# tarepan/VectorQuantizedCPC

Hardware: AMD Instinct MI355X
Metric: audio samples/sec (WaveRNN-style decode, convert.py path: encode + generate) (higher is better)
Workload: dtype f32

## Files before the change

### include/vqcpc.h

```cpp
#ifndef VQCPC_H
#define VQCPC_H

#include <stdint.h>

#ifdef __cplusplus
extern "C" {
#endif

#define VQCPC_ABI_VERSION 1

typedef enum {
    VQCPC_OK = 0,
    VQCPC_ERR_INVALID = -1,
    VQCPC_ERR_HIP = -2,
    VQCPC_ERR_NO_DEVICE = -3,
    VQCPC_ERR_ALLOC = -4
} vqcpc_status;

int vqcpc_abi_version(void);
const char *vqcpc_last_error(void);

int vqcpc_device_count(void);


// ... 71 lines not shown
typedef struct vqcpc_vocoder vqcpc_vocoder;

int vqcpc_vocoder_create(const vqcpc_vocoder_weights *w, vqcpc_vocoder **out);
void vqcpc_vocoder_destroy(vqcpc_vocoder *voc);

int vqcpc_vocoder_generate(vqcpc_vocoder *voc, const int64_t *idx, const int64_t *speaker,
                           int B, int Tc, const int *n_codes, uint64_t seed, uint32_t utt_base,
                           const uint32_t *utt_ids, float *wav, int64_t *mulaw, int max_steps,
                           void *stream);

typedef struct vqcpc_vocoder_stream vqcpc_vocoder_stream;
int vqcpc_vocoder_stream_open(vqcpc_vocoder *voc, const int64_t *idx, const int64_t *speaker, int B, int Tc,
                              const int *n_codes, uint64_t seed, uint32_t utt_base, const uint32_t *utt_ids,
                              vqcpc_vocoder_stream **out, void *stream);
int vqcpc_vocoder_stream_next(vqcpc_vocoder_stream *st, int n_samples, float *wav, int64_t *mulaw, void *stream);
int vqcpc_vocoder_stream_redo(vqcpc_vocoder_stream *st, float *wav, int64_t *mulaw, void *stream);
int vqcpc_vocoder_stream_position(const vqcpc_vocoder_stream *st, int64_t *done, int64_t *total);
void vqcpc_vocoder_stream_close(vqcpc_vocoder_stream *st);

int vqcpc_vocoder_logits(vqcpc_vocoder *voc, const int64_t *x, const int64_t *idx,
                         const int64_t *speaker, int B, int Tc, int Ts, float *logits,
                         void *stream);

int vqcpc_vocoder_nll(vqcpc_vocoder *voc, const int64_t *audio, const int64_t *idx, const int64_t *speaker,
                      int B, int Tc, int L, const int *n_codes, const int *n_audio,
                      double *nll_sum, int64_t *n_scored, int64_t *n_correct, float *nll, void *stream);

int vqcpc_vocoder_glue(vqcpc_vocoder *voc, const int64_t *idx, const int64_t *speaker, int B, int Tc, float *series,
                       void *stream);

int vqcpc_vocoder_condition(vqcpc_vocoder *voc, const int64_t *idx, const int64_t *speaker,
                            int B, int Tc, float *cond, void *stream);

int vqcpc_vocoder_set_option(vqcpc_vocoder *voc, const char *name, int value);

int vqcpc_vocoder_check(vqcpc_vocoder *voc);

int vqcpc_vocoder_last_path(vqcpc_vocoder *voc);

int vqcpc_vocoder_plan(int xcd, int xcm, int xcm_min, int xcm_max, int xcd_slots, int xcm_slots, int slots,
                       const int *n_samples, int B, int *path, int *slots_used, int64_t *longest);

int vqcpc_vocoder_last_slots(vqcpc_vocoder *voc);

int vqcpc_vocoder_workspace_bytes(vqcpc_vocoder *voc, uint64_t *bytes);

int vqcpc_vocoder_last_timing(vqcpc_vocoder *voc, float *loop_ms, int *n_steps);


typedef struct vqcpc_melfront vqcpc_melfront;
int vqcpc_melfront_create(int sr, int n_fft, int n_mels, int hop, int win, float fmin, float preemph,
                          float top_db, vqcpc_melfront **out);
void vqcpc_melfront_destroy(vqcpc_melfront *f);
int vqcpc_melfront_frames(const vqcpc_melfront *f, int n_samples);
int vqcpc_melfront_run(vqcpc_melfront *f, const float *wav, const int *lens, int B, int Lmax, float *mel,
                       void *stream);


typedef struct vqcpc_resampler vqcpc_resampler;
int vqcpc_resampler_create(int sr_in, int sr_out, vqcpc_resampler **out);
void vqcpc_resampler_destroy(vqcpc_resampler *r);
int vqcpc_resampler_out_len(const vqcpc_resampler *r, int n_in);
int vqcpc_resampler_run(vqcpc_resampler *r, const float *wav_in, const int *lens_in, int B, int Lin_max,
                        float *wav_out, int Lout_max, void *stream);


// ... 16 lines not shown
```

### vectorquantizedcpc_amd/_lib.py

```python
import ctypes as C
import os

_HERE = os.path.dirname(os.path.abspath(__file__))
LIB_PATH = os.path.join(_HERE, "libvqcpc_hip.so")

SYMBOLS = [
    "vqcpc_abi_version", "vqcpc_last_error", "vqcpc_device_count",
    "vqcpc_encoder_create", "vqcpc_encoder_destroy", "vqcpc_encoder_encode",
    "vqcpc_encoder_forward_stats", "vqcpc_encoder_context", "vqcpc_encoder_stage", "vqcpc_encoder_vq_encode", "vqcpc_encoder_set_option", "vqcpc_encoder_last_schedule",
    "vqcpc_cpc_create", "vqcpc_cpc_destroy", "vqcpc_cpc_score",
    "vqcpc_encoder_check", "vqcpc_vocoder_check", "vqcpc_vocoder_last_path", "vqcpc_vocoder_last_slots", "vqcpc_vocoder_workspace_bytes", "vqcpc_vocoder_plan",
    "vqcpc_vocoder_create", "vqcpc_vocoder_destroy", "vqcpc_vocoder_generate",
    "vqcpc_vocoder_logits", "vqcpc_vocoder_nll", "vqcpc_vocoder_condition", "vqcpc_vocoder_glue", "vqcpc_vocoder_set_option",
    "vqcpc_vocoder_last_timing", "vqcpc_vocoder_kernel_times",
    "vqcpc_vocoder_stream_open", "vqcpc_vocoder_stream_next", "vqcpc_vocoder_stream_redo", "vqcpc_vocoder_stream_position",
    "vqcpc_vocoder_stream_close",
    "vqcpc_melfront_create", "vqcpc_melfront_destroy", "vqcpc_melfront_frames", "vqcpc_melfront_run",
    "vqcpc_loudness_create", "vqcpc_loudness_destroy", "vqcpc_loudness_blocks", "vqcpc_loudness_integrated",
    "vqcpc_loudness_normalize",
    "vqcpc_resampler_create", "vqcpc_resampler_destroy", "vqcpc_resampler_out_len", "vqcpc_resampler_run",
]


class EncoderWeights(C.Structure):
    _fields_ = [("conv_weight", C.c_void_p), ("ln_weight", C.c_void_p * 5), ("ln_bias", C.c_void_p * 5),
                ("fc_weight", C.c_void_p * 4), ("out_weight", C.c_void_p), ("out_bias", C.c_void_p),
                ("codebook", C.c_void_p), ("rnn_w_ih", C.c_void_p), ("rnn_w_hh", C.c_void_p),
                ("rnn_b_ih", C.c_void_p), ("rnn_b_hh", C.c_void_p),
                ("in_channels", C.c_int), ("channels", C.c_int), ("n_embeddings", C.c_int),
                ("z_dim", C.c_int), ("c_dim", C.c_int)]


class CPCWeights(C.Structure):
    _fields_ = [("weight", C.c_void_p * 16), ("bias", C.c_void_p * 16),
                ("n_steps", C.c_int), ("n_speakers", C.c_int), ("n_utterances", C.c_int), ("n_negatives", C.c_int),
                ("z_dim", C.c_int), ("c_dim", C.c_int)]


class VocoderWeights(C.Structure):
    _fields_ = [("code_embedding", C.c_void_p), ("speaker_embedding", C.c_void_p),
                ("prenet_w_ih", (C.c_void_p * 2) * 2), ("prenet_w_hh", (C.c_void_p * 2) * 2),
                ("prenet_b_ih", (C.c_void_p * 2) * 2), ("prenet_b_hh", (C.c_void_p * 2) * 2),
                ("ar_embedding", C.c_void_p), ("ar_w_ih", C.c_void_p), ("ar_w_hh", C.c_void_p),
                ("ar_b_ih", C.c_void_p), ("ar_b_hh", C.c_void_p),
                ("fc1_weight", C.c_void_p), ("fc1_bias", C.c_void_p), ("fc2_weight", C.c_void_p), ("fc2_bias", C.c_void_p),
                ("n_codes", C.c_int), ("dz", C.c_int), ("n_speakers", C.c_int), ("ds", C.c_int), ("Hp", C.c_int),
# ... 15 lines not shown
    lib = C.CDLL(LIB_PATH)
    vp, i32, i64p = C.c_void_p, C.c_int, C.c_void_p
    lib.vqcpc_abi_version.restype = i32
    lib.vqcpc_last_error.restype = C.c_char_p
    lib.vqcpc_device_count.restype = i32
    lib.vqcpc_encoder_create.argtypes = [C.POINTER(EncoderWeights), C.POINTER(vp)]
    lib.vqcpc_encoder_destroy.argtypes = [vp]
    lib.vqcpc_encoder_destroy.restype = None
    lib.vqcpc_encoder_encode.argtypes = [vp, vp, i32, i32, i32, vp, vp, i64p, vp, vp]
    lib.vqcpc_encoder_forward_stats.argtypes = [vp, vp, vp, i64p, i32, vp, vp, vp, vp]
    lib.vqcpc_encoder_context.argtypes = [vp, vp, i32, i32, vp, vp]
    lib.vqcpc_encoder_stage.argtypes = [vp, vp, i32, i32, i32, i32, vp, vp]
    lib.vqcpc_encoder_vq_encode.argtypes = [vp, vp, i32, vp, i64p, vp]
    lib.vqcpc_encoder_set_option.argtypes = [vp, C.c_char_p, i32]
    lib.vqcpc_encoder_check.argtypes = [vp]
    lib.vqcpc_encoder_last_schedule.argtypes = [vp]
    lib.vqcpc_cpc_create.argtypes = [C.POINTER(CPCWeights), C.POINTER(vp)]
    lib.vqcpc_cpc_destroy.argtypes = [vp]
    lib.vqcpc_cpc_destroy.restype = None
    lib.vqcpc_cpc_score.argtypes = [vp, vp, vp, i32, i64p, i64p, C.c_uint64, C.c_uint32, vp, vp, vp, vp, vp, vp]
    lib.vqcpc_vocoder_check.argtypes = [vp]
    lib.vqcpc_vocoder_last_path.argtypes = [vp]
    lib.vqcpc_vocoder_last_slots.argtypes = [vp]
    lib.vqcpc_vocoder_workspace_bytes.argtypes = [vp, C.POINTER(C.c_uint64)]
    lib.vqcpc_vocoder_plan.argtypes = [i32] * 7 + [C.POINTER(C.c_int), i32, C.POINTER(C.c_int), C.POINTER(C.c_int), C.POINTER(C.c_int64)]
    lib.vqcpc_vocoder_create.argtypes = [C.POINTER(VocoderWeights), C.POINTER(vp)]
    lib.vqcpc_vocoder_destroy.argtypes = [vp]
    lib.vqcpc_vocoder_destroy.restype = None
    lib.vqcpc_vocoder_generate.argtypes = [vp, i64p, i64p, i32, i32, C.POINTER(C.c_int), C.c_uint64, C.c_uint32,
                                           C.POINTER(C.c_uint32), vp, i64p, i32, vp]
    lib.vqcpc_vocoder_logits.argtypes = [vp, i64p, i64p, i64p, i32, i32, i32, vp, vp]
    lib.vqcpc_vocoder_nll.argtypes = [vp, i64p, i64p, i64p, i32, i32, i32, C.POINTER(C.c_int), C.POINTER(C.c_int), vp, i64p, i64p, vp, vp]
    lib.vqcpc_vocoder_condition.argtypes = [vp, i64p, i64p, i32, i32, vp, vp]
    lib.vqcpc_vocoder_glue.argtypes = [vp, i64p, i64p, i32, i32, vp, vp]
    lib.vqcpc_vocoder_set_option.argtypes = [vp, C.c_char_p, i32]
    lib.vqcpc_vocoder_last_timing.argtypes = [vp, C.POINTER(C.c_float), C.POINTER(C.c_int)]
    lib.vqcpc_vocoder_kernel_times.argtypes = [vp, i32, C.POINTER(C.c_float), vp]
    lib.vqcpc_vocoder_stream_open.argtypes = [vp, i64p, i64p, i32, i32, C.POINTER(C.c_int), C.c_uint64, C.c_uint32,
                                              C.POINTER(C.c_uint32), C.POINTER(vp), vp]
    lib.vqcpc_vocoder_stream_next.argtypes = [vp, i32, vp, i64p, vp]
    lib.vqcpc_vocoder_stream_redo.argtypes = [vp, vp, i64p, vp]
    lib.vqcpc_vocoder_stream_position.argtypes = [vp, C.POINTER(C.c_int64), C.POINTER(C.c_int64)]
    lib.vqcpc_vocoder_stream_close.argtypes = [vp]
    lib.vqcpc_vocoder_stream_close.restype = None
    lib.vqcpc_melfront_create.argtypes = [i32, i32, i32, i32, i32, C.c_float, C.c_float, C.c_float, C.POINTER(vp)]
    lib.vqcpc_melfront_destroy.argtypes = [vp]
    lib.vqcpc_melfront_destroy.restype = None
    lib.vqcpc_melfront_frames.argtypes = [vp, i32]
    lib.vqcpc_melfront_run.argtypes = [vp, vp, C.POINTER(C.c_int), i32, i32, vp, vp]
    lib.vqcpc_loudness_create.argtypes = [i32, C.POINTER(vp)]
    lib.vqcpc_loudness_destroy.argtypes = [vp]
    lib.vqcpc_loudness_destroy.restype = None
    lib.vqcpc_loudness_blocks.argtypes = [vp, i32]
    lib.vqcpc_loudness_integrated.argtypes = [vp, vp, C.POINTER(C.c_int), i32, i32, vp, vp, vp]
    lib.vqcpc_loudness_normalize.argtypes = [vp, vp, C.POINTER(C.c_int), i32, i32, vp, vp, vp]
    lib.vqcpc_resampler_create.argtypes = [i32, i32, C.POINTER(vp)]
    lib.vqcpc_resampler_destroy.argtypes = [vp]
    lib.vqcpc_resampler_destroy.restype = None
    lib.vqcpc_resampler_out_len.argtypes = [vp, i32]
    lib.vqcpc_resampler_run.argtypes = [vp, vp, C.POINTER(C.c_int), i32, i32, vp, i32, vp]
    lib.vqcpc_probe_gates.argtypes = [vp, i32, vp, vp]
    _lib = lib
    return lib


def check(rc: int):
# ... 58 lines not shown
```

### vectorquantizedcpc_amd/csrc/common.h

```cpp
#pragma once
#include <hip/hip_runtime.h>
#include <stdint.h>
#include <stddef.h>
#include "../../include/vqcpc.h"

void vq_set_error(const char *fmt, ...) __attribute__((format(printf, 1, 2)));
int vq_require_gfx950();

#define HIP_TRY(expr)                                                                      \
    do {                                                                                   \
        hipError_t e_ = (expr);                                                            \
        if (e_ != hipSuccess) {                                                            \
            vq_set_error("%s failed: %s (%s:%d)", #expr, hipGetErrorString(e_), __FILE__,  \
                         __LINE__);                                                        \
            return VQCPC_ERR_HIP;                                                          \
        }                                                                                  \
    } while (0)

#define VQ_REQUIRE(cond, ...)                   \
    do {                                        \
        if (!(cond)) {                          \
            vq_set_error(__VA_ARGS__);          \
            return VQCPC_ERR_INVALID;           \
        }                                       \
// ... 8 lines not shown
    void *p = nullptr;
    size_t cap = 0;
    int reserve(size_t bytes) {
        if (bytes <= cap) return VQCPC_OK;
        if (p) (void)hipFree(p);
        p = nullptr; cap = 0;
        hipError_t e = hipMalloc(&p, bytes);
        if (e != hipSuccess) {
            vq_set_error("hipMalloc(%zu) failed: %s", bytes, hipGetErrorString(e));
            return VQCPC_ERR_ALLOC;
        }
        cap = bytes;
        return VQCPC_OK;
    }
    void release() { if (p) (void)hipFree(p); p = nullptr; cap = 0; }
    template <class T> T **fresh() { release(); return (T **)&p; }
    template <class T> T *as() const { return (T *)p; }
};
template <class T> struct DevPtr : DevBuf {
    DevPtr() = default;
    DevPtr(const DevPtr &) = delete;
    DevPtr &operator=(const DevPtr &) = delete;
    ~DevPtr() { release(); }
    operator T *() const { return (T *)p; }
};

int vq_gemm_chain(const float *A, int lda, const float *W, const float *bias, float *Y, int ldy,
                  int M, int N, int K, int KC, hipStream_t s);

int vq_gemm_chain_ex(const float *A, int lda, const float *W, const float *bias, float *Y, int ldy,
                     int M, int N, int K, int KC, int relu, int ydiv, int ystride, int yoff, int ylim, hipStream_t s);

int vq_build_wfrag(const float *W, int ldw, int n_rg, int K, int ksplit, int rowmode, int H, float **out);
int vq_bigru_scan(const float *Wf, const float *b_hh, const float *Gi, float *hbuf, float *out, const int *len, const int *row0,
                  int H, int B, int T, hipStream_t s);
struct LstmPlan;
int vq_lstm_plan_create(const float *w_ih, const float *w_hh, const float *b_ih, const float *b_hh,
                        int D, int H, LstmPlan **out);
void vq_lstm_plan_destroy(LstmPlan *p);
int vq_lstm_run(LstmPlan *p, const float *x, int B, int T, float *out, hipStream_t s);
int vq_lstm_set_persistent(LstmPlan *p, int value);
int vq_lstm_set_debug(LstmPlan *p, int drop_step, int timeout_ms);
int vq_lstm_check(LstmPlan *p);
```

### vectorquantizedcpc_amd/csrc/scan.hip

```cpp
#include "common.h"
#include "ar_shared.h"
#include <math.h>

__global__ void build_wfrag_kernel(const float *__restrict__ W, int ldw, float *__restrict__ Wf, int n_rg,
                                   int K, int ksplit, int rowmode, int H) {
    const int SW = K / 16 / ksplit;
    const size_t total = (size_t)n_rg * ksplit * SW * 64;
    const size_t id = (size_t)blockIdx.x * blockDim.x + threadIdx.x;
    if (id >= total) return;
    const int lane = (int)(id & 63);
    size_t r = id >> 6;
    const int s = (int)(r % SW); r /= SW;
    const int w = (int)(r % ksplit);
    const int rg = (int)(r / ksplit);
    const int i = lane & 15, kq = lane >> 4, S = w * SW + s;
    int row;
    if (rowmode == 0) row = 16 * rg + i;
    else if (rowmode == 8) row = i < 8 ? 8 * rg + i : -1;
    else if (rowmode == 16) row = (rg % 3) * H + 16 * (rg / 3) + i;
    else row = (i >> 2) < rowmode ? (i >> 2) * H + 4 * rg + (i & 3) : -1;
    float4 v = make_float4(0.f, 0.f, 0.f, 0.f);
    if (row >= 0) v = *(const float4 *)(W + (size_t)row * ldw + 16 * S + 4 * kq);
    ((float4 *)Wf)[id] = v;
}
// ... 61 lines not shown
    __syncthreads();
    if (act) {
        float hn;
        if (G == 3) {
            const float r = sigmoidf_(g0 + (gate[u][b] + bh0));
            const float z = sigmoidf_(g1 + (gate[4 + u][b] + bh1));
            const float n = tanhf(g2 + r * (gate[8 + u][b] + bh2));
            hn = (1.0f - z) * n + z * hold;
        } else {
            const float ig = sigmoidf_(g0 + gate[u][b]), fg = sigmoidf_(g1 + gate[4 + u][b]);
            const float gg = tanhf(g2 + gate[8 + u][b]), og = sigmoidf_(g3 + gate[12 + u][b]);
            const float cn = fg * cold + ig * gg;
            p.cbuf[(size_t)dir * hsz + hi] = cn;
            hn = og * tanhf(cn);
        }
        hout[hi] = hn;
        p.out[((p.row0 ? (size_t)p.row0[bg] : (size_t)bg * p.T) + tpos) * (p.ndir * H) + (size_t)dir * H + unit] = hn;
    }
}

template <int G>
static int launch_seq(const SeqP &p, int step, hipStream_t s) {
    const int SW = p.H / 64;
    dim3 grid(p.H / 4, p.ndir, p.nbt), blk(256);
    switch (SW) {
#define CASE(n) case n: hipLaunchKernelGGL((seq_step_kernel<G, n>), grid, blk, 0, s, p, step); break;
        CASE(1) CASE(2) CASE(4) CASE(8)
#undef CASE
        default: vq_set_error("recurrent step: hidden size %d unsupported (64, 128, 256 and 512 are built)", p.H); return VQCPC_ERR_INVALID;
    }
    return VQCPC_OK;
}

int vq_bigru_scan(const float *Wf, const float *b_hh, const float *Gi, float *hbuf, float *out, const int *len, const int *row0,
                  int H, int B, int T, hipStream_t s) {
    const int nbt = (B + 15) / 16;
    HIP_TRY(hipMemsetAsync(hbuf, 0, (size_t)2 * 2 * nbt * H * 16 * sizeof(float), s));
    SeqP q{};
    q.Wf = Wf; q.b_hh = b_hh; q.Gi = Gi; q.hbuf = hbuf;
    q.out = out; q.len = len; q.row0 = row0; q.H = H; q.nbt = nbt; q.B = B; q.T = T; q.ndir = 2;
    for (int t = 0; t < T; ++t) TRY(launch_seq<3>(q, t, s));
    return VQCPC_OK;
}

__global__ void add_vec_kernel(const float *a, const float *b, float *o, int n) {
    const int i = blockIdx.x * blockDim.x + threadIdx.x;
    if (i < n) o[i] = a[i] + b[i];
}

struct LstmPlan {
    int D, H;
    float *w_ih = nullptr, *bias = nullptr, *Wf = nullptr;
    float *w_hh = nullptr;
    DevBuf gi, hbuf, cbuf, px;
    unsigned *abort_host = nullptr;
    int persistent = -1;
    bool pending = false;
    int dbg_drop_step = -1;
    int timeout_ms = 1000;
};
static int lstm_persist_launch(LstmPlan *p, int T, float *out, hipStream_t s);
void vq_lstm_plan_destroy(LstmPlan *p) {
    if (!p) return;
    if (p->w_ih) (void)hipFree(p->w_ih);
    if (p->bias) (void)hipFree(p->bias);
    if (p->Wf) (void)hipFree(p->Wf);
    if (p->w_hh) (void)hipFree(p->w_hh);
    if (p->abort_host) (void)hipHostFree(p->abort_host);
// ... 45 lines not shown
    HIP_TRY(hipMemsetAsync(p->hbuf.p, 0, 2 * hsz, s));
    HIP_TRY(hipMemsetAsync(p->cbuf.p, 0, hsz, s));
    SeqP q{};
    q.Wf = p->Wf; q.Gi = p->gi.as<float>(); q.hbuf = p->hbuf.as<float>(); q.cbuf = p->cbuf.as<float>();
    q.out = out; q.len = nullptr; q.H = H; q.nbt = nbt; q.B = B; q.T = T; q.ndir = 1;
    for (int t = 0; t < T; ++t) TRY(launch_seq<4>(q, t, s));
    HIP_TRY(hipGetLastError());
    return VQCPC_OK;
}

__device__ __forceinline__ int ps_perm(int k) { return (k & ~15) | ((k & 3) << 2) | ((k >> 2) & 3); }

template <int NS>
__device__ __forceinline__ float ps_chain(const float (&w)[8 * NS], const float4 *hb, int kw, int c0) {
    float acc = 0.f;
#pragma unroll
    for (int s = 0; s < NS; ++s) {
        const float4 h0 = hb[(kw * NS + s) * 4 + c0], h1 = hb[(kw * NS + s) * 4 + c0 + 2];
        acc = __builtin_fmaf(w[8 * s + 0], h0.x, acc); acc = __builtin_fmaf(w[8 * s + 1], h0.y, acc);
        acc = __builtin_fmaf(w[8 * s + 2], h0.z, acc); acc = __builtin_fmaf(w[8 * s + 3], h0.w, acc);
        acc = __builtin_fmaf(w[8 * s + 4], h1.x, acc); acc = __builtin_fmaf(w[8 * s + 5], h1.y, acc);
        acc = __builtin_fmaf(w[8 * s + 6], h1.z, acc); acc = __builtin_fmaf(w[8 * s + 7], h1.w, acc);
    }
    return acc;
}
__device__ __forceinline__ float ps_combine(float acc, int lane) {
    (void)lane;
    const float other = PS_DPP(acc, 0xB1);
    const float q = acc + other;
    const float q1 = PS_DPP(q, 0x4E);
    const float q2 = PS_DPP(q, 0x104);
    const float q3 = PS_DPP(q, 0x106);
    return ((q + q1) + q2) + q3;
}

#define PS_PAD 16
__device__ __forceinline__ int ps_slot(int idx, int per_blk) { return (idx / per_blk) * PS_PAD + idx % per_blk; }

template <int N>
__device__ __forceinline__ bool ps_sweep(const u64 *g, int lane, int per_blk, unsigned tag, unsigned (&val)[N], unsigned *abort_flag,
                                         u64 ticks = 100000000ull) {
    const u64 t0 = __builtin_amdgcn_s_memrealtime();
    int slot[N];
#pragma unroll
    for (int j = 0; j < N; ++j) slot[j] = ps_slot(lane + 64 * j, per_blk);
    for (unsigned spins = 0;; ++spins) {
        bool ok = true;
#pragma unroll
        for (int j = 0; j < N; ++j) {
            const u64 x = ps_load(g + slot[j]);
            val[j] = (unsigned)x;
            ok &= (unsigned)(x >> 32) == tag;
        }
        if (__all(ok)) return true;
        if ((spins & 63) == 63) {
            const bool late = __builtin_amdgcn_s_memrealtime() - t0 > ticks;
            if (late || __hip_atomic_load(abort_flag, __ATOMIC_RELAXED, __HIP_MEMORY_SCOPE_SYSTEM) != 0u) {
                if (late && lane == 0) __hip_atomic_store(abort_flag, 1u, __ATOMIC_RELAXED, __HIP_MEMORY_SCOPE_SYSTEM);
                return false;
            }
        }
        __builtin_amdgcn_s_sleep(1);
    }
}

#define LP_NW 32
// ... 96 lines not shown
```

### vectorquantizedcpc_amd/csrc/vocoder_host.hip

```cpp
#include "vocoder_internal.h"
#include <math.h>
#include <stdio.h>
#include <limits.h>


__global__ void quads_build_kernel(const float *__restrict__ src, float4 *__restrict__ dst, int rows, int H) {
    const size_t id = (size_t)blockIdx.x * blockDim.x + threadIdx.x;
    if (id >= (size_t)rows * H) return;
    const int unit = (int)(id % H);
    const size_t row = id / H;
    const float *s = src + row * 3 * H + unit;
    dst[row * H + unit] = make_float4(s[0], s[H], s[2 * H], 0.f);
}

__global__ void glue_kernel(const int64_t *__restrict__ idx, const int64_t *__restrict__ spk,
                            const float *__restrict__ ce, const float *__restrict__ se, float *__restrict__ out,
                            int B, int Tc, int dz, int ds, int n_codes, int n_spk, unsigned *status, unsigned status_tag,
                            const int *__restrict__ frames, const int *__restrict__ row0) {
    const int F = dz + ds;
    size_t i = (size_t)blockIdx.x * blockDim.x + threadIdx.x;
    if (i >= (size_t)B * 2 * Tc * F) return;
    const int f = (int)(i % F);
    const size_t r = i / F;
    const int t2 = (int)(r % (2 * Tc)), b = (int)(r / (2 * Tc));
// ... 135 lines not shown
    *out = nullptr;
    TRY(vq_require_gfx950());
    VQ_REQUIRE(w->bits_mu_law >= 8 && w->bits_mu_law <= 10 && w->n_cls == (1 << w->bits_mu_law),
               "vocoder: bits_mu_law must be 8 (config.py:15), 9 or 10 with n_cls = 2^bits (got %d, %d)", w->bits_mu_law, w->n_cls);
    VQ_REQUIRE(w->Hf >= 256 && w->Hf <= 1024 && w->Hf % 256 == 0, "vocoder: size_h_fc must be 256 (config.py:77), 512, 768 or 1024 (got %d)", w->Hf);
    VQ_REQUIRE((w->dz + w->ds) % 32 == 0 && w->Hp % 64 == 0 && w->Hp <= 1024, "vocoder: dz+ds %% 32 and Hp %% 64 required");
    VQ_REQUIRE(w->de % 32 == 0, "vocoder: size_i_embed_ar %% 32 required (got %d)", w->de);
    VQ_REQUIRE(w->Hr == 512 || w->Hr == 896 || w->Hr == 1024, "vocoder: size_h_rnn %d: the per-sample kernels are built for 512, 896 "
               "(config.py:76) and 1024", w->Hr);
    VQ_REQUIRE(w->Hp == 64 || w->Hp == 128 || w->Hp == 256 || w->Hp == 512, "vocoder: dim_voc_latent / 2 = %d: the prenet scan is built "
               "for 64, 128 (config.py:68), 256 and 512", w->Hp);
    VQ_REQUIRE(w->upsample_t > 0, "vocoder: upsample_t must be positive");
    vqcpc_vocoder *v = new vqcpc_vocoder();
    int rc = vocoder_create_impl(w, v);
    if (rc != VQCPC_OK) { vqcpc_vocoder_destroy(v); return rc; }
    *out = v;
    return VQCPC_OK;
}

enum { OPT_BOOL = 1, OPT_GRAPHS = 2, OPT_EVEN = 4 };
struct OptSpec { const char *name; int vqcpc_vocoder::*field; int lo, hi, flags; };
static const OptSpec k_options[] = {
    {"use_graph", &vqcpc_vocoder::use_graph, 0, 1, OPT_BOOL},
    {"steps_per_graph", &vqcpc_vocoder::steps_per_graph, 2, 4096, OPT_GRAPHS | OPT_EVEN},
    {"big_min_tiles", &vqcpc_vocoder::big_min_tiles, 0, INT_MAX, OPT_GRAPHS},
    {"two_groups", &vqcpc_vocoder::two_groups, 0, 1, OPT_BOOL},
    {"fuse_fc2", &vqcpc_vocoder::fuse_fc2, 0, 1, OPT_BOOL | OPT_GRAPHS},
    {"handoff_timeout_ms", &vqcpc_vocoder::handoff_timeout_ms, 1, 10000, OPT_GRAPHS},
    {"handoff_debug_drop_step", &vqcpc_vocoder::handoff_debug_drop_step, INT_MIN, INT_MAX, OPT_GRAPHS},
    {"xcd", &vqcpc_vocoder::xcd, -1, 1, 0},
    {"xcd_slots", &vqcpc_vocoder::xcd_slots, 1, 8 * XD_MAX_BX, 0},
    {"xcd_agent_stores", &vqcpc_vocoder::xcd_agent_stores, 0, 1, OPT_BOOL},
    {"xcm", &vqcpc_vocoder::xcm, -1, 1, 0},
    {"xcm_min", &vqcpc_vocoder::xcm_min, 0, 65536, 0},
    {"xcm_max", &vqcpc_vocoder::xcm_max, 0, 1 << 20, 0},
    {"xcm_slots", &vqcpc_vocoder::xcm_slots, 1, 8 * XM_BX, 0},
    {"xcd_timeout_ms", &vqcpc_vocoder::xcd_timeout_ms, 1, 10000, 0},
    {"xcd_debug_drop_step", &vqcpc_vocoder::xcd_debug_drop_step, INT_MIN, INT_MAX, 0},
    {"xcd_debug_misplace", &vqcpc_vocoder::xcd_debug_misplace, 0, 1, OPT_BOOL},
    {"tf_chunk_replays", &vqcpc_vocoder::tf_chunk_replays, 1, 64, 0},
    {"slots", &vqcpc_vocoder::n_slots, 0, 65536, 0},
};

extern "C" int vqcpc_vocoder_set_option(vqcpc_vocoder *v, const char *name, int value) {
    VQ_REQUIRE(v && name, "vqcpc_vocoder_set_option: null argument");
    for (const OptSpec &o : k_options) {
        if (strcmp(name, o.name)) continue;
        if (o.flags & OPT_BOOL) value = value != 0;
        VQ_REQUIRE(value >= o.lo && value <= o.hi && !((o.flags & OPT_EVEN) && value % 2), "%s must be %sin [%d, %d]", name,
                   (o.flags & OPT_EVEN) ? "even and " : "", o.lo, o.hi);
        if ((o.flags & OPT_GRAPHS) && value != v->*o.field) clear_graphs(v);
        v->*o.field = value;
        if (o.field == &vqcpc_vocoder::xcd) { v->fell_back = false; v->placement_misses = 0; }
        return VQCPC_OK;
    }
    vq_set_error("unknown option %s", name);
    return VQCPC_ERR_INVALID;
}

constexpr int REARM_CLEAN = 16;
static void fall_back(vqcpc_vocoder *v) {
    if (!v->fell_back) { v->saved_xcd = v->xcd; v->saved_fuse_fc2 = v->fuse_fc2; }
    v->fell_back = true; v->clean_calls = 0; v->xcd = 0;
}
static int status_check(vqcpc_vocoder *v, bool synced) {
    if (!v->status_pending) return VQCPC_OK;
// ... 60 lines not shown
    *bytes = n;
    return VQCPC_OK;
}

extern "C" int vqcpc_vocoder_last_timing(vqcpc_vocoder *v, float *loop_ms, int *n_steps) {
    VQ_REQUIRE(v && loop_ms && n_steps, "vqcpc_vocoder_last_timing: null argument");
    TRY(status_check(v, true));
    HIP_TRY(hipEventElapsedTime(loop_ms, v->ev0, v->ev1));
    *n_steps = v->last_steps;
    return VQCPC_OK;
}

static int run_condition(vqcpc_vocoder *v, const int64_t *idx, const int64_t *spk, int B, int Tc,
                         const int *frames_dev, const int *row0_dev, size_t n_rows, float *cond_out, hipStream_t s) {
    const auto &d = v->d;
    const int F = d.dz + d.ds, Hp = d.Hp, dl = 2 * Hp, T2 = 2 * Tc, nbt = (B + 15) / 16;
    const size_t rows = row0_dev ? (n_rows ? n_rows : 1) : (size_t)B * T2;
    TRY(v->series.reserve(rows * F * sizeof(float)));
    TRY(v->gi.reserve(rows * 6 * Hp * sizeof(float)));
    TRY(v->out0.reserve(rows * dl * sizeof(float)));
    const size_t hsz = (size_t)2 * nbt * Hp * 16 * sizeof(float);
    TRY(v->hseq.reserve(2 * hsz));
    const size_t ng = (size_t)B * T2 * F;
    hipLaunchKernelGGL(glue_kernel, dim3((unsigned)((ng + 255) / 256)), dim3(256), 0, s, idx, spk, v->code_emb,
                       v->spk_emb, v->series.as<float>(), B, Tc, d.dz, d.ds, d.n_codes, d.n_speakers, v->status_dev, v->epoch << 8,
                       frames_dev, row0_dev);
    v->status_pending = true;
    for (int l = 0; l < 2; ++l) {
        const float *xin = l == 0 ? v->series.as<float>() : v->out0.as<float>();
        const int I = l == 0 ? F : dl;
        float *xout = l == 0 ? v->out0.as<float>() : cond_out;
        TRY(vq_gemm_chain(xin, I, v->p_wih[l], v->p_bih[l], v->gi.as<float>(), 6 * Hp, (int)rows, 6 * Hp, I, I, s));
        if (frames_dev && !row0_dev) HIP_TRY(hipMemsetAsync(xout, 0, rows * dl * sizeof(float), s));
        TRY(vq_bigru_scan(v->p_wf[l], v->p_bhh[l], v->gi.as<float>(), v->hseq.as<float>(), xout, frames_dev, row0_dev, Hp, B, T2, s));
    }
    HIP_TRY(hipGetLastError());
    return VQCPC_OK;
}

static int tf_chunk_gemms(vqcpc_vocoder *v, int B, int Ts, int CH, int chunk, float *logits, hipStream_t s) {
    const auto &d = v->d;
    const int M = B * CH;
    TRY(vq_gemm_chain_ex(v->hall.as<float>(), d.Hr, v->w_fc1, v->b_fc1, v->a1c.as<float>(), d.Hf, M, d.Hf, d.Hr, d.Hr,
                         1, 0, 0, 0, 0, s));
    TRY(vq_gemm_chain_ex(v->a1c.as<float>(), d.Hf, v->w_fc2, v->b_fc2, logits, d.n_cls, M, d.n_cls, d.Hf, d.Hf,
                         0, CH, Ts, chunk * CH, Ts, s));
    return VQCPC_OK;
}

struct NllCall {
    const int64_t *audio;
    int L;
    std::vector<int> slen;
    float *nll;
    double *nll_sum; int64_t *n_scored, *n_correct;
};

static int tf_chunk_nll(vqcpc_vocoder *v, int B, int CH, int chunk, const NllCall &nc, hipStream_t s) {
    NllHead h{};
    h.hall = v->hall.as<float>(); h.w1 = v->w_fc1; h.b1 = v->b_fc1; h.w2 = v->w_fc2; h.b2 = v->b_fc2;
    h.audio = nc.audio; h.slen = v->nll_len.as<int>(); h.nll = nc.nll; h.part = v->nll_part.as<NllPart>();
    h.status = v->status_dev; h.status_tag = v->epoch << 8;
    h.B = B; h.L = nc.L; h.CH = CH; h.t0 = chunk * CH; h.Hr = v->d.Hr;
    return vq_tf_nll_chunk(h, nc.nll_sum, nc.n_scored, nc.n_correct, s);
}
int run_resident(vqcpc_vocoder *v, const CallPlan &cp, int T2, unsigned long long seed, float *wav, int64_t *mulaw, hipStream_t s, const Resume *rs) {
    VQ_REQUIRE(!rs || cp.dp.path == 2, "vocoder stream: chunks do not run on the matrix-core decoders");
// ... 292 lines not shown
            if (pass == 1) HIP_TRY(hipEventRecord(v->ev0, s));
            const int n = pass == 0 ? 20 : reps;
            for (int i = 0; i < n; ++i) {
                if (which == 2) { launch_fc2_step(a, m, call, 0, c.nbt, s); continue; }
                if (which == 1) { TRY(launch_fc1_step(a, m, call, 0, c.nbt, s)); continue; }
                const int period = c.max_t > 5 ? (c.max_t - 3) / 2 : 1;
                const int tl = m.fused ? 1 + 2 * (fresh++ % period) : 0;
                TRY(launch_gru_step(a, m, call, tl, c.nbt, m.fused ? nf : 0, s));
            }
        }
        HIP_TRY(hipEventRecord(v->ev1, s));
        HIP_TRY(hipStreamSynchronize(s));
        float ms = 0.f;
        HIP_TRY(hipEventElapsedTime(&ms, v->ev0, v->ev1));
        out_us[which] = ms * 1e3f / (float)reps;
    }
    out_us[3] = (float)(c.nbt * 16);
    out_us[4] = m.fused ? (tbig ? 5.f : 4.f) : (c.nbt == 1 ? 0.f : (tbig ? 2.f : 1.f));
    return VQCPC_OK;
}

extern "C" int vqcpc_vocoder_glue(vqcpc_vocoder *v, const int64_t *idx, const int64_t *speaker, int B, int Tc, float *series,
                                  void *stream) {
    VQ_REQUIRE(v && idx && speaker && series && B > 0 && Tc > 0, "vqcpc_vocoder_glue: bad argument");
    const auto &d = v->d;
    const size_t ng = (size_t)B * 2 * Tc * (d.dz + d.ds);
    hipLaunchKernelGGL(glue_kernel, dim3((unsigned)((ng + 255) / 256)), dim3(256), 0, (hipStream_t)stream, idx, speaker, v->code_emb,
                       v->spk_emb, series, B, Tc, d.dz, d.ds, d.n_codes, d.n_speakers, v->status_dev, v->epoch << 8, nullptr, nullptr);
    v->status_pending = true;
    HIP_TRY(hipGetLastError());
    return VQCPC_OK;
}

extern "C" int vqcpc_vocoder_condition(vqcpc_vocoder *v, const int64_t *idx, const int64_t *speaker, int B, int Tc,
                                       float *cond, void *stream) {
    VQ_REQUIRE(v && idx && speaker && cond && B > 0 && Tc > 0, "vqcpc_vocoder_condition: bad argument");
    return run_condition(v, idx, speaker, B, Tc, nullptr, nullptr, 0, cond, (hipStream_t)stream);
}
```

### vectorquantizedcpc_amd/csrc/vocoder_internal.h

```cpp
#pragma once
#include "common.h"
#include "ar_shared.h"
#include "ar_xcd.h"
#include "ar_step.h"
#include "nll.h"
#include <string.h>
#include <map>
#include <vector>

struct HostStage {
    char *p = nullptr;
    size_t cap = 0, used = 0;
    hipEvent_t ev = nullptr;
    bool pending = false;
    int begin(size_t need) {
        if (!ev) HIP_TRY(hipEventCreateWithFlags(&ev, hipEventDisableTiming));
        if (pending) { HIP_TRY(hipEventSynchronize(ev)); pending = false; }
        if (need > cap) {
            if (p) (void)hipHostFree(p);
            p = nullptr; cap = 0;
            const size_t want = need + need / 2 + 4096;
            HIP_TRY(hipHostMalloc((void **)&p, want, hipHostMallocDefault));
            cap = want;
        }
// ... 34 lines not shown
        DevBuf har, a1, cand_s, cand_k, slot_tab, cur, gcur, candg;
        std::map<int, hipGraphExec_t> graphs;
        const void *baked[8] = {nullptr, nullptr, nullptr, nullptr, nullptr, nullptr, nullptr, nullptr};
    } grp[2];
    int two_groups = 1;
    hipStream_t side_stream = nullptr;
    hipEvent_t ev_fork = nullptr, ev_join = nullptr;
    DevBuf series, gi, out0, cond, gcond, gbase, hseq, len;
    DevBuf hall, a1c;
    DevBuf nll_part, nll_len;
    unsigned *status_host = nullptr;
    unsigned *status_dev = nullptr;
    HostStage stage;
    DevPtr<float> w_hh;
    int fuse_fc2 = 1;
    bool status_pending = false;
    unsigned epoch = 0;
    int last_slots = 0;
    int placement_misses = 0;
    bool fell_back = false;
    int saved_xcd = -1, saved_fuse_fc2 = 1, clean_calls = 0;
    int handoff_timeout_ms = 250;
    int handoff_debug_drop_step = -1;
    int xcd = -1;
    int xcd_slots = XCD_SLOTS_DEFAULT;
    int xcd_agent_stores = 0;
    int xcd_timeout_ms = 250;
    int xcd_debug_drop_step = -1;
    int xcm = -1;
    int xcm_min = XCM_MIN_DEFAULT, xcm_max = XCM_MAX_DEFAULT;
    int xcm_slots = XCM_SLOTS_DEFAULT;
    int xcd_debug_misplace = 0;
    DevBuf xd_x, xd_segs;
    int tf_chunk_replays = 4;
    int use_graph = 1, steps_per_graph = 160;
    int n_slots = 0;
    int big_min_tiles = 5;
    bool big_attr_set = false;
    hipStream_t cap_stream = nullptr;
    hipEvent_t ev0 = nullptr, ev1 = nullptr;
    int last_steps = 0;
    ArCall last_call{};
    ArModel last_model{};
    int last_path = 1;
};


struct PlanOpts {
    int xcd, xcm, xcm_min, xcm_max, xcd_slots, xcm_slots, n_slots; bool supported;
    int upsample_t, steps_per_graph, fuse_fc2, big_min_tiles, two_groups, use_graph;
};

struct DecodePlan {
    int path = 0, xs = 0, bxt = 0;
    long longest = 0;
    std::vector<std::vector<XdSeg>> lists;
    std::vector<long> xend;
};

struct UttLayout {
    std::vector<int> lens;
    std::vector<unsigned> utt;
    std::vector<int> gbase;
    long grows = 0;
};

// ... 21 lines not shown
```

### vectorquantizedcpc_amd/network_vocoder.py

```python
import ctypes as C
import numbers
from dataclasses import dataclass, field

import torch
import torch.nn as nn
from torch import Tensor

from . import _lib

MISSING = "???"


@dataclass
class ConfPreNet:
    num_layers: int = 2
    bidirectional: bool = True


@dataclass
class ConfWaveAR:
    size_i_embed_ar: int = 256
    size_h_rnn: int = 896
    size_h_fc: int = 256

# ... 280 lines not shown
        na, nc = host_ints(lengths, "lengths"), host_ints(n_codes, "n_codes")
        dev = z.device
        nll_sum = torch.empty(B, dtype=torch.float64, device=dev)
        n_scored = torch.empty(B, dtype=torch.int64, device=dev)
        n_correct = torch.empty(B, dtype=torch.int64, device=dev)
        nll = torch.empty(B, L - 1, device=dev) if per_sample else None
        with torch.cuda.device(dev):
            _lib.check(_lib.load().vqcpc_vocoder_nll(
                self._native(), audio.data_ptr(), z.data_ptr(), speaker.data_ptr(), B, Tc, L, nc, na, nll_sum.data_ptr(),
                n_scored.data_ptr(), n_correct.data_ptr(), nll.data_ptr() if per_sample and L > 1 else None,
                _lib.current_stream()))
            self.check()
        return VocoderNLL(nll_sum, n_scored, n_correct, nll)

    @torch.no_grad()
    def glue(self, z: Tensor, speaker: Tensor) -> Tensor:
        z, speaker = self._prep(z, speaker)
        B, Tc = z.shape
        out = torch.empty(B, 2 * Tc, self.conf.dim_i_embedding + self.conf.dim_speaker_embedding, device=z.device)
        with torch.cuda.device(z.device):
            _lib.check(_lib.load().vqcpc_vocoder_glue(self._native(), z.data_ptr(), speaker.data_ptr(), B, Tc, out.data_ptr(),
                                                      _lib.current_stream()))
            self.check()
        return out

    @torch.no_grad()
    def condition(self, z: Tensor, speaker: Tensor) -> Tensor:
        z, speaker = self._prep(z, speaker)
        B, Tc = z.shape
        out = torch.empty(B, 2 * Tc, self.conf.rnnms.dim_voc_latent, device=z.device)
        with torch.cuda.device(z.device):
            _lib.check(_lib.load().vqcpc_vocoder_condition(self._native(), z.data_ptr(), speaker.data_ptr(), B, Tc,
                                                           out.data_ptr(), _lib.current_stream()))
            self.check()
        return out


@dataclass
class VocoderNLL:
    nll_sum: Tensor
    n_scored: Tensor
    n_correct: Tensor
    nll: object = None

    @property
    def loss(self) -> Tensor:
        return self.nll_sum.sum() / self.n_scored.sum()


class VocoderStream:

    def __init__(self, voc, handle, st, B, chunk, device, return_mulaw):
        self._voc, self._handle, self._st = voc, handle, st
        self._B, self._chunk, self._device, self._return_mulaw = B, chunk, device, return_mulaw
        self._final = None

    def __iter__(self):
        return self

    @property
    def position(self):
        if self._st is None:
            return self._final
        done, total = C.c_int64(), C.c_int64()
        _lib.check(_lib.load().vqcpc_vocoder_stream_position(self._st, C.byref(done), C.byref(total)))
        return int(done.value), int(total.value)
# ... 50 lines not shown
```

Baseline: 9.051 million.

## Add resident per-sequence BiGRU prenet scan kernel with register-held weights

Adds a persistent bidirectional GRU scan kernel for H=128 in which each workgroup owns one sequence and direction, keeps its recurrent weights in registers, and double-buffers the input-gate projections through shared memory in blocks of 8 timesteps. It is used by default when 2*B is at most 256 workgroups, replacing the tiled scan that keeps hidden state in a global buffer and needs that buffer memset first. The aim is to remove global round-trips and launch/sync overhead in the prenet conditioning recurrence. It also adds a gcond debug API and a prenet_resident option. The trade-off is fewer workgroups (only 2*B), so occupancy is low when B is small.

```diff
diff --git a/include/vqcpc.h b/include/vqcpc.h
--- a/include/vqcpc.h
+++ b/include/vqcpc.h
@@ -127,6 +127,9 @@
 int vqcpc_vocoder_condition(vqcpc_vocoder *voc, const int64_t *idx, const int64_t *speaker,
                             int B, int Tc, float *cond, void *stream);
 
+int vqcpc_vocoder_gcond(vqcpc_vocoder *voc, const int64_t *idx, const int64_t *speaker, int B, int Tc, const int *n_codes,
+                        float *gcond, void *stream);
+
 int vqcpc_vocoder_set_option(vqcpc_vocoder *voc, const char *name, int value);
 
 int vqcpc_vocoder_check(vqcpc_vocoder *voc);
diff --git a/vectorquantizedcpc_amd/_lib.py b/vectorquantizedcpc_amd/_lib.py
--- a/vectorquantizedcpc_amd/_lib.py
+++ b/vectorquantizedcpc_amd/_lib.py
@@ -11,7 +11,7 @@
     "vqcpc_cpc_create", "vqcpc_cpc_destroy", "vqcpc_cpc_score",
     "vqcpc_encoder_check", "vqcpc_vocoder_check", "vqcpc_vocoder_last_path", "vqcpc_vocoder_last_slots", "vqcpc_vocoder_workspace_bytes", "vqcpc_vocoder_plan",
     "vqcpc_vocoder_create", "vqcpc_vocoder_destroy", "vqcpc_vocoder_generate",
-    "vqcpc_vocoder_logits", "vqcpc_vocoder_nll", "vqcpc_vocoder_condition", "vqcpc_vocoder_glue", "vqcpc_vocoder_set_option",
+    "vqcpc_vocoder_logits", "vqcpc_vocoder_nll", "vqcpc_vocoder_condition", "vqcpc_vocoder_gcond", "vqcpc_vocoder_glue", "vqcpc_vocoder_set_option",
     "vqcpc_vocoder_last_timing", "vqcpc_vocoder_kernel_times",
     "vqcpc_vocoder_stream_open", "vqcpc_vocoder_stream_next", "vqcpc_vocoder_stream_redo", "vqcpc_vocoder_stream_position",
     "vqcpc_vocoder_stream_close",
@@ -93,6 +93,7 @@
     lib.vqcpc_vocoder_logits.argtypes = [vp, i64p, i64p, i64p, i32, i32, i32, vp, vp]
     lib.vqcpc_vocoder_nll.argtypes = [vp, i64p, i64p, i64p, i32, i32, i32, C.POINTER(C.c_int), C.POINTER(C.c_int), vp, i64p, i64p, vp, vp]
     lib.vqcpc_vocoder_condition.argtypes = [vp, i64p, i64p, i32, i32, vp, vp]
+    lib.vqcpc_vocoder_gcond.argtypes = [vp, i64p, i64p, i32, i32, C.POINTER(C.c_int), vp, vp]
     lib.vqcpc_vocoder_glue.argtypes = [vp, i64p, i64p, i32, i32, vp, vp]
     lib.vqcpc_vocoder_set_option.argtypes = [vp, C.c_char_p, i32]
     lib.vqcpc_vocoder_last_timing.argtypes = [vp, C.POINTER(C.c_float), C.POINTER(C.c_int)]
diff --git a/vectorquantizedcpc_amd/csrc/common.h b/vectorquantizedcpc_amd/csrc/common.h
--- a/vectorquantizedcpc_amd/csrc/common.h
+++ b/vectorquantizedcpc_amd/csrc/common.h
@@ -64,8 +64,9 @@
                      int M, int N, int K, int KC, int relu, int ydiv, int ystride, int yoff, int ylim, hipStream_t s);
 
 int vq_build_wfrag(const float *W, int ldw, int n_rg, int K, int ksplit, int rowmode, int H, float **out);
+constexpr int BIGRU_RESIDENT_MAX_WG = 256;
 int vq_bigru_scan(const float *Wf, const float *b_hh, const float *Gi, float *hbuf, float *out, const int *len, const int *row0,
-                  int H, int B, int T, hipStream_t s);
+                  int H, int B, int T, int resident, hipStream_t s);
 struct LstmPlan;
 int vq_lstm_plan_create(const float *w_ih, const float *w_hh, const float *b_ih, const float *b_hh,
                         int D, int H, LstmPlan **out);
diff --git a/vectorquantizedcpc_amd/csrc/scan.hip b/vectorquantizedcpc_amd/csrc/scan.hip
--- a/vectorquantizedcpc_amd/csrc/scan.hip
+++ b/vectorquantizedcpc_amd/csrc/scan.hip
@@ -117,8 +117,13 @@
     return VQCPC_OK;
 }
 
+static int bigru_resident_launch(const float *Wf, const float *b_hh, const float *Gi, float *out, const int *len, const int *row0,
+                                 int B, int T, hipStream_t s);
+
 int vq_bigru_scan(const float *Wf, const float *b_hh, const float *Gi, float *hbuf, float *out, const int *len, const int *row0,
-                  int H, int B, int T, hipStream_t s) {
+                  int H, int B, int T, int resident, hipStream_t s) {
+    if (H == 128 && (resident > 0 || (resident < 0 && 2 * B <= BIGRU_RESIDENT_MAX_WG)))
+        return bigru_resident_launch(Wf, b_hh, Gi, out, len, row0, B, T, s);
     const int nbt = (B + 15) / 16;
     HIP_TRY(hipMemsetAsync(hbuf, 0, (size_t)2 * 2 * nbt * H * 16 * sizeof(float), s));
     SeqP q{};
@@ -230,6 +235,106 @@
     const float q2 = PS_DPP(q, 0x104);
     const float q3 = PS_DPP(q, 0x106);
     return ((q + q1) + q2) + q3;
+}
+
+#define BR_H 128
+#define BR_BLK 8
+struct BigruResP {
+    const float *Wf;
+    const float *b_hh;
+    const float *Gi;
+    float *out;
+    const int *len;
+    const int *row0;
+    int T;
+};
+__device__ __forceinline__ float br_weight(const float *Wf, int gate, int unit, int k) {
+    return Wf[((size_t)((unit >> 2) * (BR_H / 16) + (k >> 4)) * 64 + ((k >> 2) & 3) * 16 + gate * 4 + (unit & 3)) * 4 + (k & 3)];
+}
+__device__ __forceinline__ float br_chain(const float (&w)[16], const float4 (&hv)[4]) {
+    float acc = 0.f;
+#pragma unroll
+    for (int s = 0; s < 2; ++s) {
+        const float4 h0 = hv[2 * s], h1 = hv[2 * s + 1];
+        acc = __builtin_fmaf(w[8 * s + 0], h0.x, acc); acc = __builtin_fmaf(w[8 * s + 1], h0.y, acc);
+        acc = __builtin_fmaf(w[8 * s + 2], h0.z, acc); acc = __builtin_fmaf(w[8 * s + 3], h0.w, acc);
+        acc = __builtin_fmaf(w[8 * s + 4], h1.x, acc); acc = __builtin_fmaf(w[8 * s + 5], h1.y, acc);
+        acc = __builtin_fmaf(w[8 * s + 6], h1.z, acc); acc = __builtin_fmaf(w[8 * s + 7], h1.w, acc);
+    }
+    return acc;
+}
+__global__ __launch_bounds__(6 * BR_H) void bigru_resident_kernel(BigruResP p) {
+    constexpr int H = BR_H, Q = 3 * H / 4;
+    __shared__ __attribute__((aligned(16))) float hb[H];
+    __shared__ __attribute__((aligned(16))) float gsum[3 * H];
+    __shared__ float4 ring[2][BR_BLK][Q];
+    const int tid = threadIdx.x, lane = tid & 63, b = blockIdx.x, dir = blockIdx.y;
+    int L = p.len ? p.len[b] : p.T;
+    L = L > p.T ? p.T : L;
+    if (L <= 0) return;
+    const size_t base = p.row0 ? (size_t)p.row0[b] : (size_t)b * p.T;
+    const float *gi = p.Gi + base * (6 * H) + (size_t)dir * 3 * H;
+    float *out = p.out + base * (2 * H) + (size_t)dir * H;
+    const int g = tid >> 3, kw = (lane & 7) >> 1, c0 = lane & 1;
+    float w[4][16];
+    {
+        const float *Wd = p.Wf + (size_t)dir * (H / 4) * (H / 16) * 64 * 4;
+#pragma unroll
+        for (int j = 0; j < 4; ++j)
+#pragma unroll
+            for (int n = 0; n < 16; ++n) w[j][n] = br_weight(Wd, g >> 5, 4 * (g & 31) + j, chain_col(2, kw, c0, n));
+    }
+    float bh0 = 0.f, bh1 = 0.f, bh2 = 0.f, hprev = 0.f;
+    if (tid < H) {
+        const float *bh = p.b_hh + (size_t)dir * 3 * H + tid;
+        bh0 = bh[0]; bh1 = bh[H]; bh2 = bh[2 * H];
+        hb[tid] = 0.f;
+    }
+    const int fj = tid / Q, fq = tid % Q;
+    auto fetch = [&](int t0) {
+        const int t = t0 + fj;
+        float4 v = make_float4(0.f, 0.f, 0.f, 0.f);
+        if (t < L) v = ((const float4 *)(gi + (size_t)(dir == 0 ? t : L - 1 - t) * (6 * H)))[fq];
+        return v;
+    };
+    float4 pf = fetch(0);
+    ring[0][fj][fq] = pf;
+    ps_barrier();
+    for (int t0 = 0; t0 < L; t0 += BR_BLK) {
+        const int slot = (t0 / BR_BLK) & 1;
+        const bool more = t0 + BR_BLK < L;
+        if (more) pf = fetch(t0 + BR_BLK);
+        const int nj = L - t0 < BR_BLK ? L - t0 : BR_BLK;
+        for (int j = 0; j < nj; ++j) {
+            const float4 *hb4 = (const float4 *)hb;
+            const float4 hv[4] = {hb4[(kw * 2) * 4 + c0], hb4[(kw * 2) * 4 + c0 + 2], hb4[(kw * 2 + 1) * 4 + c0], hb4[(kw * 2 + 1) * 4 + c0 + 2]};
+            float v[4];
+#pragma unroll
+            for (int r = 0; r < 4; ++r) v[r] = ps_combine(br_chain(w[r], hv), lane);
+            if ((lane & 7) == 0) *(float4 *)&gsum[4 * g] = make_float4(v[0], v[1], v[2], v[3]);
+            ps_barrier();
+            if (tid < H) {
+                const float *gr = (const float *)ring[slot][j];
+                const float r = sigmoidf_(gr[tid] + (gsum[tid] + bh0));
+                const float z = sigmoidf_(gr[H + tid] + (gsum[H + tid] + bh1));
+                const float n = tanhf(gr[2 * H + tid] + r * (gsum[2 * H + tid] + bh2));
+                const float hn = (1.0f - z) * n + z * hprev;
+                hprev = hn;
+                hb[ps_perm(tid)] = hn;
+                const int t = t0 + j;
+                out[(size_t)(dir == 0 ? t : L - 1 - t) * (2 * H) + tid] = hn;
+            }
+            ps_barrier();
+        }
+        if (more) ring[slot ^ 1][fj][fq] = pf;
+    }
+}
+static int bigru_resident_launch(const float *Wf, const float *b_hh, const float *Gi, float *out, const int *len, const int *row0,
+                                 int B, int T, hipStream_t s) {
+    BigruResP q{Wf, b_hh, Gi, out, len, row0, T};
+    hipLaunchKernelGGL(bigru_resident_kernel, dim3(B, 2), dim3(6 * BR_H), 0, s, q);
+    HIP_TRY(hipGetLastError());
+    return VQCPC_OK;
 }
 
 #define PS_PAD 16
diff --git a/vectorquantizedcpc_amd/csrc/vocoder_host.hip b/vectorquantizedcpc_amd/csrc/vocoder_host.hip
--- a/vectorquantizedcpc_amd/csrc/vocoder_host.hip
+++ b/vectorquantizedcpc_amd/csrc/vocoder_host.hip
@@ -191,6 +191,7 @@
     {"xcd_slots", &vqcpc_vocoder::xcd_slots, 1, 8 * XD_MAX_BX, 0},
     {"xcd_agent_stores", &vqcpc_vocoder::xcd_agent_stores, 0, 1, OPT_BOOL},
     {"xcm", &vqcpc_vocoder::xcm, -1, 1, 0},
+    {"prenet_resident", &vqcpc_vocoder::prenet_resident, -1, 1, 0},
     {"xcm_min", &vqcpc_vocoder::xcm_min, 0, 65536, 0},
     {"xcm_max", &vqcpc_vocoder::xcm_max, 0, 1 << 20, 0},
     {"xcm_slots", &vqcpc_vocoder::xcm_slots, 1, 8 * XM_BX, 0},
@@ -317,7 +318,7 @@
         float *xout = l == 0 ? v->out0.as<float>() : cond_out;
         TRY(vq_gemm_chain(xin, I, v->p_wih[l], v->p_bih[l], v->gi.as<float>(), 6 * Hp, (int)rows, 6 * Hp, I, I, s));
         if (frames_dev && !row0_dev) HIP_TRY(hipMemsetAsync(xout, 0, rows * dl * sizeof(float), s));
-        TRY(vq_bigru_scan(v->p_wf[l], v->p_bhh[l], v->gi.as<float>(), v->hseq.as<float>(), xout, frames_dev, row0_dev, Hp, B, T2, s));
+        TRY(vq_bigru_scan(v->p_wf[l], v->p_bhh[l], v->gi.as<float>(), v->hseq.as<float>(), xout, frames_dev, row0_dev, Hp, B, T2, v->prenet_resident, s));
     }
     HIP_TRY(hipGetLastError());
     return VQCPC_OK;
@@ -676,6 +677,19 @@
     return VQCPC_OK;
 }
 
+extern "C" int vqcpc_vocoder_gcond(vqcpc_vocoder *v, const int64_t *idx, const int64_t *speaker, int B, int Tc, const int *n_codes,
+                                   float *gcond, void *stream) {
+    VQ_REQUIRE(v && idx && speaker && gcond && B > 0 && Tc > 0, "vqcpc_vocoder_gcond: bad argument");
+    hipStream_t s = (hipStream_t)stream;
+    CallPlan cp;
+    TRY(plan_call(plan_opts(v), B, Tc, n_codes, false, 0, 0, 0, nullptr, cp));
+    TRY(begin_call(v, cp, B));
+    TRY(run_conditioning(v, cp, idx, speaker, B, Tc, v->cond, v->gcond, v->gbase, s));
+    if (cp.grows > 0)
+        HIP_TRY(hipMemcpyAsync(gcond, v->gcond.p, (size_t)cp.grows * 3 * v->d.Hr * sizeof(float), hipMemcpyDeviceToDevice, s));
+    return VQCPC_OK;
+}
+
 extern "C" int vqcpc_vocoder_condition(vqcpc_vocoder *v, const int64_t *idx, const int64_t *speaker, int B, int Tc,
                                        float *cond, void *stream) {
     VQ_REQUIRE(v && idx && speaker && cond && B > 0 && Tc > 0, "vqcpc_vocoder_condition: bad argument");
diff --git a/vectorquantizedcpc_amd/csrc/vocoder_internal.h b/vectorquantizedcpc_amd/csrc/vocoder_internal.h
--- a/vectorquantizedcpc_amd/csrc/vocoder_internal.h
+++ b/vectorquantizedcpc_amd/csrc/vocoder_internal.h
@@ -90,6 +90,7 @@
     int xcm_slots = XCM_SLOTS_DEFAULT;
     int xcd_debug_misplace = 0;
     DevBuf xd_x, xd_segs;
+    int prenet_resident = -1;
     int tf_chunk_replays = 4;
     int use_graph = 1, steps_per_graph = 160;
     int n_slots = 0;
diff --git a/vectorquantizedcpc_amd/network_vocoder.py b/vectorquantizedcpc_amd/network_vocoder.py
--- a/vectorquantizedcpc_amd/network_vocoder.py
+++ b/vectorquantizedcpc_amd/network_vocoder.py
@@ -336,6 +336,18 @@
         with torch.cuda.device(z.device):
             _lib.check(_lib.load().vqcpc_vocoder_condition(self._native(), z.data_ptr(), speaker.data_ptr(), B, Tc,
                                                            out.data_ptr(), _lib.current_stream()))
+            self.check()
+        return out
+
+    @torch.no_grad()
+    def gcond(self, z: Tensor, speaker: Tensor, *, n_codes=None) -> Tensor:
+        z, speaker = self._prep(z, speaker)
+        B, Tc = z.shape
+        nc = [Tc] * B if n_codes is None else [int(v) for v in n_codes]
+        out = torch.empty(2 * sum(nc), 3 * self.conf.rnnms.wave_ar.size_h_rnn, device=z.device)
+        with torch.cuda.device(z.device):
+            _lib.check(_lib.load().vqcpc_vocoder_gcond(self._native(), z.data_ptr(), speaker.data_ptr(), B, Tc, (C.c_int * B)(*nc),
+                                                       out.data_ptr(), _lib.current_stream()))
             self.check()
         return out
 
```

Result: no change. 9.142 million (median of 6 runs) (+1.0%).
